# zengjianping/openpose

Hardware: AMD Instinct MI355X
Metric: frames/sec whole-node, BODY_25 -1x368 @1280x720, 1/2/4/8 GPU + CPU ref (higher is better)
Workload: dtype fp16

## Files before the change

openpose_amd/csrc/host/context.h:

```cpp
#pragma once
#include <hip/hip_runtime.h>

#include <map>
#include <memory>
#include <tuple>
#include <vector>

#include "../common.h"
#include "../kernels/kernels.h"
#include "pose_model.h"

struct opk_render_layer;
struct opk_render_heat;

namespace opk {

void cubic_tables(int s, int d, int* ofs, float* coef);

struct Context {
    int device = 0;
    hipStream_t stream = nullptr;
    bool owns_stream = false;

    struct Tables { DevBuf buf; const int* yofs; const float* ycoef; const int* xofs; const float* xcoef; };
    std::map<std::tuple<int, int, int, int>, std::unique_ptr<Tables>> resize_tables;
    const Tables& tables(int sh, int sw, int dh, int dw);

    struct PoseDev { DevBuf buf; PafPairTable t; };
    std::map<int, std::unique_ptr<PoseDev>> pose_dev;
    const PafPairTable& pose_table(int model);

    DevBuf warp_weights[2];
    const short* warp_weight_table(bool cubic);
    struct WarpAxes { DevBuf buf; const int* x; const int* y; };
    std::map<std::tuple<uint64_t, int, int>, std::unique_ptr<WarpAxes>> warp_axes;
    const WarpAxes& warp_axis_tables(double scale, int dw, int dh);

    struct RenderDev { DevBuf buf; const unsigned* pairs; const float* scales; const float* colors;
                       int npairs, nscales, ncolors; };
    std::map<int, std::unique_ptr<RenderDev>> render_dev;
    const RenderDev& render_table(int which);
    DevBuf render_geom;
    DevBuf frames_offsets, frames_keypoints;
    std::vector<int> frames_offsets_host;

    DevBuf scratch_scores;
    DevBuf nms_scratch;
    int* nms_candidates(int frames, int parts);
    HostBuf host_peaks, host_scores;

    std::vector<hipStream_t> side_streams;
    void add_side_stream(hipStream_t s) { side_streams.push_back(s); }
    void remove_side_stream(hipStream_t s)
    {
        for (size_t i = 0; i < side_streams.size(); ++i)
            if (side_streams[i] == s) {
                side_streams.erase(side_streams.begin() + (long)i);
// ... 32 lines not shown
```

openpose_amd/csrc/host/input.cpp:

```cpp
#include "input.h"

#include <cmath>
#include <cstring>
#include <vector>

#include "../common.h"
#include "../kernels/kernels.h"
#include "context.h"

namespace opk {

namespace {
constexpr int kInterBits = 5, kInterTab = 1 << kInterBits;
constexpr int kAbBits = 10, kAbScale = 1 << kAbBits;
constexpr int kCoefScale = 1 << 15;

int round_half_even(double v) { return (int)std::lrint(v); }
int round_half_even(float v) { return (int)std::lrintf(v); }

int positive_round(float v) { return (int)(v + 0.5f); }
int positive_round(double v) { return (int)(v + 0.5f); }
}

void scale_and_size(int in_w, int in_h, int net_w, int net_h, float dyn, int scale_number,
                    double scale_gap, double* scales, int* sizes)
{
    OPK_CHECK_ARG(in_w > 0 && in_h > 0, "Wrong input element (empty cvInputData).");
    OPK_CHECK_ARG(scale_number >= 1, "scale_number must be >= 1");
    if (net_w <= 0 || net_h <= 0) {
// ... 96 lines not shown
        OPK_HIP(hipStreamSynchronize(stream));
    }
    return static_cast<const short*>(b.ptr);
}

const Context::WarpAxes& Context::warp_axis_tables(double scale, int dw, int dh)
{
    uint64_t bits;
    std::memcpy(&bits, &scale, sizeof bits);
    const auto key = std::make_tuple(bits, dw, dh);
    auto it = warp_axes.find(key);
    if (it != warp_axes.end()) return *it->second;
    const bool cubic = scale > 1.;
    std::vector<int> host(2 * (size_t)(dw + dh));
    warp_axis_table(scale, dw, cubic, host.data());
    warp_axis_table(scale, dh, cubic, host.data() + 2 * dw);
    auto t = std::make_unique<WarpAxes>();
    int* dev = static_cast<int*>(t->buf.get(host.size() * sizeof(int)));
    OPK_HIP(hipMemcpyAsync(dev, host.data(), host.size() * sizeof(int), hipMemcpyHostToDevice,
                           stream));
    OPK_HIP(hipStreamSynchronize(stream));
    t->x = dev;
    t->y = dev + 2 * dw;
    auto& ref = *t;
    warp_axes.emplace(key, std::move(t));
    return ref;
}

void cvmat_to_input(Context* ctx, float* dst, const uint8_t* src, int n, int sw, int sh,
                    size_t step, double scale, int dw, int dh, int normalize, hipStream_t stream)
{
    OPK_CHECK_ARG(dst && src, "NULL buffer");
    OPK_CHECK_ARG(n > 0 && sw > 0 && sh > 0 && dw > 0 && dh > 0, "empty frame or net input");
    OPK_CHECK_ARG(scale > 0 && std::isfinite(scale), "scale must be positive");
    ctx->bind();
    const bool cubic = scale > 1.;
    const short* w = ctx->warp_weight_table(cubic);
    const auto& ax = ctx->warp_axis_tables(scale, dw, dh);
    launch_cvmat_to_input(dst, src, n, sh, sw, step ? step : (size_t)sw * 3, dh, dw, ax.x, ax.y, w,
                          cubic ? 4 : 2, normalize, stream ? stream : ctx->stream);
}

}
```

openpose_amd/csrc/host/net.cpp:

```cpp
#include "net.h"

#include "caffemodel.h"

#include <algorithm>
#include <cmath>
#include <cstdlib>
#include <set>

namespace opk {

namespace {
int round_up(int v, int m) { return (v + m - 1) / m * m; }
int pick_bn(int cout)
{
    if (cout <= 32) return 32;
    if (cout <= 64) return 64;
    if (cout <= 96) return 96;
    return 128;
}
}

NetHip::NetHip(Context* ctx, std::vector<LayerDesc> layers, const std::string& output_blob)
    : ctx_(ctx), output_blob_(output_blob)
{
// ... 678 lines not shown
        }
        a.split = S.csplit[ci] ? 1 : 0;
        a.wscale = S.csplit[ci] ? c.wscale : 1.f;
        a.in_lo = S.csplit[ci] && use3 && !S.query[ci].xhi ? S.base_lo[c.in.buf] : nullptr;
        for (size_t q = 0; q < pools_.size(); ++q)
            if (S.poolfused[q] && pool_conv_[q] == (int)ci) {
                a.pool = 1;
                a.ndst = 1;
                a.dst[0] = ptr[pools_[q].out_buf];
                a.dst_lo[0] = S.csplit[ci] ? S.base_lo[pools_[q].out_buf] : nullptr;
                a.dst_cs[0] = bufs_[pools_[q].out_buf].cs;
                a.dst_coff[0] = 0;
            }
        if (c.out32_coff >= 0) {
            OPK_CHECK_ARG(c.level == out_level_, c.info.name + ": output at another resolution");
            a.out32 = S.out32;
            a.out32_c = out_c_;
            a.out32_coff = c.out32_coff;
        }
    }
    return &S;
}

void NetHip::forward(const float* input, int n, int h, int w)
{
    forward_on(input, n, h, w, ctx_->stream, true);
}

float* NetHip::select_output(int n, int h, int w, bool alternate)
{
    OPK_CHECK_ARG(n > 0 && h > 0 && w > 0, "empty input");
    ctx_->bind();
    ShapePlan& S = *shape_plan(n, h, w, ctx_->stream);
    if (alternate) {
        if (!S.out32_alt) {
            const size_t bytes = (size_t)n * out_c_ * S.lh[out_level_] * S.lw[out_level_] * 4;
            S.out32_alt = static_cast<float*>(S.out_mem_alt.get(bytes));
        }
        S.alt = !S.alt;
    }
    return S.out();
}

void NetHip::note_reader(const float* out, hipEvent_t ev)
{
    for (auto& r : readers_)
        if (r.first == out) {
            r.second = ev;
            return;
        }
    readers_.emplace_back(out, ev);
}

void NetHip::forget_reader_events(const hipEvent_t* evs, int n)
{
    for (size_t i = readers_.size(); i-- > 0;)
        for (int k = 0; k < n; ++k)
            if (readers_[i].second == evs[k]) {
                readers_.erase(readers_.begin() + (long)i);
                break;
            }
}

void NetHip::prepare(int n, int h, int w)
{
    OPK_CHECK_ARG(n > 0 && h > 0 && w > 0, "empty input");
    ctx_->bind();
    (void)shape_plan(n, h, w, ctx_->stream);
}

void NetHip::forward_on(const float* input, int n, int h, int w, hipStream_t st, bool timed)
{
    OPK_CHECK_ARG(input && n > 0 && h > 0 && w > 0, "empty input");
    OPK_CHECK_ARG(ready(), "weights not loaded for every convolution");
    ctx_->bind();
    ShapePlan& S = *shape_plan(n, h, w, st);
    cur_ = &S;
    for (const auto& r : readers_)
        if (r.first == S.out()) OPK_HIP(hipStreamWaitEvent(st, r.second, 0));
    if (timed) timer_.begin(st);
    forward_launches(S, input, n, h, w, st);
    if (timed) timer_.end(st);
}

void NetHip::blob(const std::string& name, int f0, int nf, float* host, int shape[4]) const
{
    read_planes(name, f0, nf, nullptr, nullptr, host, shape, nullptr);
}

void NetHip::blob_planes(const std::string& name, int f0, int nf, float* hi, float* lo, int shape[4],
                         int* has_lo) const
{
    read_planes(name, f0, nf, hi, lo, nullptr, shape, has_lo);
}

void NetHip::read_planes(const std::string& name, int f0, int nf, float* hi, float* lo, float* sum,
                         int shape[4], int* has_lo) const
{
    OPK_CHECK_ARG(cur_ != nullptr, "no forward yet");
    const auto it = blob_loc_.find(name);
    OPK_CHECK_ARG(it != blob_loc_.end(), "no blob named " + name);
    const BlobLoc& L = it->second;
    const ShapePlan& S = *cur_;
    OPK_CHECK_ARG(f0 >= 0 && nf > 0 && f0 + nf <= S.n, "frames out of range");
// ... 23 lines not shown
    const size_t frame_elems = (size_t)Hp * Wp * cs;
    std::vector<uint16_t> raw(frame_elems * nf), rlo(twin ? frame_elems * nf : 0);
    OPK_HIP(hipMemcpy(raw.data(), S.base[L.buf] + (size_t)f0 * frame_elems, raw.size() * 2,
                      hipMemcpyDeviceToHost));
    if (twin)
        OPK_HIP(hipMemcpy(rlo.data(), S.base_lo[L.buf] + (size_t)f0 * frame_elems, rlo.size() * 2,
                          hipMemcpyDeviceToHost));
    for (int f = 0; f < nf; ++f)
        for (int y = 0; y < H; ++y)
            for (int x = 0; x < W; ++x) {
                const size_t at = f * frame_elems + ((size_t)(y + B) * Wp + x + B) * cs + L.coff;
                const uint16_t* src = raw.data() + at;
                for (int c = 0; c < L.ch; ++c) {
                    const size_t o = ((size_t)f * L.ch + c) * hw + (size_t)y * W + x;
                    const float vh = (float)__builtin_bit_cast(_Float16, src[c]);
                    const float vl = twin ? (float)__builtin_bit_cast(_Float16, rlo[at + c]) : 0.f;
                    if (hi) hi[o] = vh;
                    if (lo) lo[o] = vl;
                    if (sum) sum[o] = vh + vl;
                }
            }
}

void NetHip::forward_launches(ShapePlan& S, const float* input, int n, int h, int w, hipStream_t st)
{
    const bool logging = dev_switch("LAUNCH_LOG", 0) != 0;
    if (logging) {
        log_.lines.clear();
        attach_launch_log(&log_);
    }
    struct Detach {
        bool on;
        ~Detach() { if (on) attach_launch_log(nullptr); }
    } detach{logging};
    forward_steps(S, input, n, h, w, st);
}

static void launch_conv3_frames(const ConvArgs& a, hipStream_t st)
{
    const int B = a.border > 0 ? a.border : 1;
    Conv3Query q = conv3_query(a);
    const int run = conv3_run_frames(q);
    if (run == a.frames) {
        launch_conv3(a, st);
        return;
    }
    const size_t frame_pos = (size_t)(a.H + 2 * B) * (a.W + 2 * B);
    const size_t dst_pos = a.pool ? (size_t)(a.H / 2 + 2 * B) * (a.W / 2 + 2 * B) : frame_pos;
    for (int f0 = 0; f0 < a.frames; f0 += run) {
        ConvArgs b = a;
        b.frames = std::min(run, a.frames - f0);
        q.frames = b.frames;
        const Conv3Plan pb = conv3_plan(q);
        b.sw = pb.sw;
        b.nstrips = pb.nstrips;
        b.M = b.frames * a.H * (a.W + 2 * B);
        b.in = a.in + f0 * frame_pos * a.in_cs;
        if (a.in_lo) b.in_lo = a.in_lo + f0 * frame_pos * a.in_cs;
        for (int d = 0; d < a.ndst; ++d) {
            b.dst[d] = a.dst[d] + f0 * dst_pos * a.dst_cs[d];
            if (a.dst_lo[d]) b.dst_lo[d] = a.dst_lo[d] + f0 * dst_pos * a.dst_cs[d];
        }
        if (a.out32) b.out32 = a.out32 + (size_t)f0 * a.out32_c * a.H * a.W;
        launch_conv3(b, st);
    }
}

void NetHip::forward_steps(ShapePlan& S, const float* input, int n, int h, int w, hipStream_t st)
{
    LaunchLog* log = launch_log();
    float* const out32 = S.out();
    const std::vector<uint16_t*>& ptr = S.base;
    const std::vector<int>& lh_ = S.lh;
    const std::vector<int>& lw_ = S.lw;
    size_t first = 0;
    if (S.fused1) {
        const ConvPlan& a = convs_[fuse1_.a];
        const ConvPlan& b = convs_[fuse1_.b];
        const PoolPlan& p = pools_[fuse1_.p];
        Conv1FusedArgs fa{};
        fa.img = input;
        fa.frames = n;
        fa.H = h;
        fa.W = w;
        fa.w1 = static_cast<const uint16_t*>(a.w.ptr);
        fa.b1 = static_cast<const float*>(a.bias.ptr);
        fa.s1 = static_cast<const float*>(a.slope.ptr);
        fa.act1 = a.info.act;
        fa.w2 = static_cast<const uint16_t*>(b.w3.ptr);
        fa.b2 = static_cast<const float*>(b.bias.ptr);
        fa.s2 = static_cast<const float*>(b.slope.ptr);
        fa.act2 = b.info.act;
        fa.out = ptr[p.out_buf];
        fa.out_cs = bufs_[p.out_buf].cs;
        fa.out_coff = 0;
        fa.OH = lh_[1];
        fa.OW = lw_[1];
        fa.actmax = a.slope01 && b.slope01 && dev_switch("EPI_MAX", 1) != 0;
        if (log) log->layer = a.info.name + "+" + b.info.name + "+pool";
        launch_conv1_fused(fa, std::min(cus_, std::max(1, dev_switch("GRID_CUS", cus_))), st);
        first = 3;
    }
    for (size_t si = first; si < steps_.size(); ++si) {
        const Step& s = steps_[si];
// ... 118 lines not shown
```

openpose_amd/csrc/host/net.h:

```cpp
#pragma once
#include <map>
#include <memory>
#include <string>
#include <vector>

#include "../kernels/conv.h"
#include "context.h"
#include "graph.h"

namespace opk {

class NetHip {
public:
    NetHip(Context* ctx, std::vector<LayerDesc> layers, const std::string& output_blob = "net_output");

    struct ConvInfo {
        std::string name;
        int cin, cout, k, act;
        std::string act_layer;
    };
    const std::vector<ConvInfo>& convs() const { return info_; }
    void set_conv(const std::string& name, const float* w, const float* b, const float* slope);
    static constexpr int kPrecisionFp16 = 0, kPrecisionSplit = 1;
    void set_precision(int precision);
    void set_precision_schedule(const int* precisions, int count);
    int conv_precision(int index) const;
    void set_small_batch(bool on);
    bool small_batch() const { return small_batch_; }
    void conv_plan(int index, int n, int h, int w, int cus, int* bm, int* bn, int* workgroups,
                   int* small) const;
    std::vector<std::string> conv_kernels(int index, int n, int h, int w, int cus) const;
    bool ready() const;
    int load_caffemodel(const std::string& path);

    void forward(const float* input, int n, int h, int w);
    void forward_on(const float* input, int n, int h, int w, hipStream_t stream, bool timed);
    void prepare(int n, int h, int w);
    void time_begin(hipStream_t s) { timer_.begin(s); }
    void time_end(hipStream_t s) { timer_.end(s); }
    float* output() const { return cur_ ? cur_->out() : nullptr; }
    float* select_output(int n, int h, int w, bool alternate);
    std::weak_ptr<void> liveness() const { return alive_; }
    void note_reader(const float* out, hipEvent_t ev);
    void forget_reader_events(const hipEvent_t* evs, int n);
    int out_channels() const { return out_c_; }
    int out_h() const { return cur_ ? cur_->lh[out_level_] : 0; }
    int out_w() const { return cur_ ? cur_->lw[out_level_] : 0; }
    int frames() const { return cur_ ? cur_->n : 0; }
    static constexpr int kMaxShapes = 8;
    double flops_per_frame(int h, int w) const;
    int border() const { return border_; }
    ~NetHip();

    void set_timing(bool on);
    void read_timing(int* count, double* total_ms);

    void blob(const std::string& name, int f0, int nf, float* host, int shape[4]) const;
    void blob_planes(const std::string& name, int f0, int nf, float* hi, float* lo, int shape[4],
                     int* has_lo) const;
// ... 36 lines not shown
        std::vector<char> headfused;
        std::vector<char> poolfused;
        std::vector<Conv3Query> query;
        std::vector<Conv3Plan> conv;
    };
    Dispatch dispatch(int n, int h, int w, int cus) const;

    struct ShapePlan : Dispatch {
        int n = 0, h = 0, w = 0;
        std::vector<std::unique_ptr<DevBuf>> mem;
        std::vector<uint16_t*> base;
        std::vector<std::unique_ptr<DevBuf>> mem_lo;
        std::vector<uint16_t*> base_lo;
        DevBuf out_mem, out_mem_alt;
        float* out32 = nullptr;
        float* out32_alt = nullptr;
        bool alt = false;
        float* out() const { return alt ? out32_alt : out32; }
        std::vector<ConvArgs> args;
        std::vector<char> use3;
    };

    void plan(const std::vector<LayerDesc>& layers);
    void forward_launches(ShapePlan& S, const float* input, int n, int h, int w, hipStream_t st);
    void forward_steps(ShapePlan& S, const float* input, int n, int h, int w, hipStream_t st);
    ShapePlan* shape_plan(int n, int h, int w, hipStream_t zero_stream = nullptr);

    Context* ctx_;
    std::string output_blob_;
    std::vector<ConvInfo> info_;
    std::vector<ConvPlan> convs_;
    std::map<std::string, int> conv_by_name_;
    std::vector<PoolPlan> pools_;
    std::vector<Step> steps_;
    std::vector<BufSpec> bufs_;
    int out_level_ = 0, out_c_ = 0, nlevels_ = 1;
    int image_buf_ = -1;
    struct Fuse1 { int a = -1, b = -1, p = -1, abuf = -1, bbuf = -1; };
    Fuse1 fuse1_;
    struct FuseHead { int a = -1, b = -1, step = -1, buf = -1; };
    std::vector<FuseHead> heads_;
    std::vector<int> pool_conv_;
    int cus_ = 256;
    bool small_batch_ = false;
    int border_ = 1;

    struct BlobLoc { int buf = -1, coff = 0, ch = 0, level = 0; bool out32 = false; };
    std::map<std::string, BlobLoc> blob_loc_;
// ... 12 lines not shown
```

openpose_amd/csrc/host/pose.cpp:

```cpp
#include "pose.h"

#include <sched.h>

#include <algorithm>
#include <chrono>
#include <cmath>
#include <cstring>
#include <exception>
#include <string>
#include <thread>

#include "../../../include/opk.h"
#include "input.h"
#include "maps.h"

namespace opk {

double resize_scale_factor(int iw, int ih, int tw, int th)
{
    const double rw = (tw - 1) / (double)(iw - 1);
    const double rh = (th - 1) / (double)(ih - 1);
    return rw < rh ? rw : rh;
}

// ... 311 lines not shown
            if (kind == KeypointExtractor::kFace) detect_faces(model_, kp_[f].data(), people_[f], parts, r);
            else detect_hands(model_, kp_[f].data(), people_[f], parts, r);
        }
        p.kp.assign((size_t)per * total * p.ex->parts() * 3, 0.f);
        const double rect_ms =
            std::chrono::duration<double, std::milli>(std::chrono::steady_clock::now() - t0).count();
        p.ex->extract(sl.raw.ptr, sl.raw.n, sl.raw.w, sl.raw.h, sl.raw.step, p.rects.data(),
                      frame_of.data(), total, p.kp.data(), true);
        ++p.batches;
        p.crops += p.ex->crops();
        p.host_ms += rect_ms + p.ex->last_host_ms();
        p.wait_ms += p.ex->last_wait_ms();
    }
    parts_valid_ = true;
}

void PoseHip::submit(const float* frames, int n, int net_h, int net_w, int prod_w, int prod_h)
{
    need_frames();
    OPK_CHECK_ARG(net_ != nullptr, "no network: use forward_net_output (poseNetOutput path)");
    OPK_CHECK_ARG(count_ < 2, "two batches already in flight: collect first");
    ctx_->bind();
    next_output(n, net_h, net_w, true);
    live_net()->forward(frames, n, net_h, net_w);
    const NetOutput o{live_net()->output(), live_net()->out_h(), live_net()->out_w()};
    submit_outputs(&o, 1, n, net_h, net_w, prod_w, prod_h, true);
}

hipStream_t PoseHip::post_stream(bool own_net)
{
    if (!own_net || ctx_->device < 0 || dev_switch("POST_STREAM", 1) == 0) {
        wait_post(ctx_->stream);
        return ctx_->stream;
    }
    if (!post_) {
        OPK_HIP(hipStreamCreateWithFlags(&post_, hipStreamNonBlocking));
        OPK_HIP(hipEventCreateWithFlags(&nets_done_, hipEventDisableTiming));
        for (auto& e : post_done_) OPK_HIP(hipEventCreateWithFlags(&e, hipEventDisableTiming));
        ctx_->add_side_stream(post_);
    }
    OPK_HIP(hipEventRecord(nets_done_, ctx_->stream));
    OPK_HIP(hipStreamWaitEvent(post_, nets_done_, 0));
    return post_;
}

void PoseHip::wait_post(hipStream_t s)
{
// ... 14 lines not shown
    OPK_CHECK_ARG(1. - (scale_number - 1) * scale_gap >= 0. && scale_gap >= 0.,
                  "All scales must be in the range [0, 1], i.e., 0 <= 1-scale_number*scale_gap <= 1");
    in_net_w_ = net_w;
    in_net_h_ = net_h;
    dyn_ = dyn;
    scale_number_ = scale_number;
    scale_gap_ = scale_gap;
}

void PoseHip::submit_frames(const uint8_t* frames, int n, int w, int h, size_t step)
{
    OPK_CHECK_ARG(net_ != nullptr, "no network: raw frames need the net");
    OPK_CHECK_ARG(frames != nullptr && n > 0 && w > 0 && h > 0, "empty frames");
    OPK_CHECK_ARG(count_ < 2, "two batches already in flight: collect first");
    OPK_CHECK_ARG(model_ != 6, "BODY_19N (DenseNet normalisation) is not supported");
    double scales[kMaxResizeSources];
    scale_and_size(w, h, in_net_w_, in_net_h_, dyn_, scale_number_, scale_gap_, scales, input_hw_);
    const float* ptrs[kMaxResizeSources];
    int hw[2 * kMaxResizeSources];
    ctx_->bind();
    for (int i = 0; i < scale_number_; ++i) {
        const int nw = input_hw_[2 * i], nh = input_hw_[2 * i + 1];
        float* x = static_cast<float*>(inputs_[i].get((size_t)n * 3 * nh * nw * sizeof(float)));
        cvmat_to_input(ctx_, x, frames, n, w, h, step, scales[i], nw, nh, 1, ctx_->stream);
        ptrs[i] = x;
        hw[2 * i] = nh;
        hw[2 * i + 1] = nw;
    }
    inputs_n_ = n;
    for (int i = 0; i < scale_number_; ++i) map_ratios_[i] = (float)scales[i];
    have_ratios_ = true;
    cur_raw_ = RawFrames{frames, n, w, h, step};
    try {
        if (scale_number_ == 1)
            submit(ptrs[0], n, hw[0], hw[1], w, h);
        else
            submit_multi(ptrs, hw, scale_number_, n, w, h);
    } catch (...) {
        have_ratios_ = false;
        cur_raw_ = RawFrames{};
        throw;
    }
    have_ratios_ = false;
    cur_raw_ = RawFrames{};
}

void PoseHip::forward_frames(const uint8_t* frames, int n, int w, int h, size_t step)
{
    OPK_CHECK_ARG(count_ == 0, "batches in flight: collect them first");
    submit_frames(frames, n, w, h, step);
    collect();
}

const float* PoseHip::net_input(int i, int* w, int* h) const
{
    OPK_CHECK_ARG(i >= 0 && i < scale_number_ && inputs_n_ > 0, "no such scale");
    if (w) *w = input_hw_[2 * i];
    if (h) *h = input_hw_[2 * i + 1];
    return static_cast<const float*>(inputs_[i].ptr);
}

void PoseHip::submit_multi(const float* const* frames, const int* net_hw, int nscales, int n,
                           int prod_w, int prod_h)
{
    need_frames();
    OPK_CHECK_ARG(net_ != nullptr, "no network: multi-scale needs the net");
    OPK_CHECK_ARG(frames && net_hw && nscales >= 1 && nscales <= kMaxResizeSources,
                  "1..8 scales");
    OPK_CHECK_ARG(count_ < 2, "two batches already in flight: collect first");
    std::vector<NetOutput> outs(nscales);
    for (int i = 0; i < nscales; ++i) OPK_CHECK_ARG(frames[i] != nullptr, "NULL scale input");
    ctx_->bind();
    bool distinct = dev_switch("MULTISCALE_STREAMS", 1) != 0;
    for (int i = 0; i < nscales && distinct; ++i)
        for (int j = 0; j < i; ++j)
            distinct = distinct && !(net_hw[2 * i] == net_hw[2 * j] && net_hw[2 * i + 1] == net_hw[2 * j + 1]);
    for (int i = 0; i < nscales; ++i) next_output(n, net_hw[2 * i], net_hw[2 * i + 1], nscales == 1 || distinct);
    if (nscales == 1 || !distinct) {
        for (int i = 0; i < nscales; ++i) {
            live_net()->forward(frames[i], n, net_hw[2 * i], net_hw[2 * i + 1]);
            outs[i] = NetOutput{live_net()->output(), live_net()->out_h(), live_net()->out_w()};
        }
    } else {
        if (!fork_) {
            OPK_HIP(hipEventCreateWithFlags(&fork_, hipEventDisableTiming));
            for (int i = 0; i < kMaxResizeSources - 1; ++i) {
                OPK_HIP(hipStreamCreateWithFlags(&scale_streams_[i], hipStreamNonBlocking));
                OPK_HIP(hipEventCreateWithFlags(&join_[i], hipEventDisableTiming));
            }
        }
        for (int i = 0; i < nscales; ++i) live_net()->prepare(n, net_hw[2 * i], net_hw[2 * i + 1]);
        hipStream_t s = ctx_->stream;
        live_net()->time_begin(s);
        OPK_HIP(hipEventRecord(fork_, s));
        live_net()->forward_on(frames[0], n, net_hw[0], net_hw[1], s, false);
        outs[0] = NetOutput{live_net()->output(), live_net()->out_h(), live_net()->out_w()};
        for (int i = 1; i < nscales; ++i) {
            OPK_HIP(hipStreamWaitEvent(scale_streams_[i - 1], fork_, 0));
            live_net()->forward_on(frames[i], n, net_hw[2 * i], net_hw[2 * i + 1], scale_streams_[i - 1],
                             false);
            outs[i] = NetOutput{live_net()->output(), live_net()->out_h(), live_net()->out_w()};
            OPK_HIP(hipEventRecord(join_[i - 1], scale_streams_[i - 1]));
        }
        for (int i = 1; i < nscales; ++i) OPK_HIP(hipStreamWaitEvent(s, join_[i - 1], 0));
        live_net()->time_end(s);
    }
    submit_outputs(outs.data(), nscales, n, net_hw[0], net_hw[1], prod_w, prod_h, true);
}

void PoseHip::submit_net_output(const float* net_out, int n, int oh, int ow, int net_h,
                                int net_w, int prod_w, int prod_h)
{
    need_frames();
    const NetOutput o{net_out, oh, ow};
    submit_outputs(&o, 1, n, net_h, net_w, prod_w, prod_h, false);
}

void PoseHip::submit_outputs(const NetOutput* outs, int nscales, int n, int net_h, int net_w,
                             int prod_w, int prod_h, bool own_net)
{
    const PoseModelInfo& m = pose_model(model_);
    const int C = m.heat_channels();
    OPK_CHECK_ARG(n > 0 && nscales >= 1 && nscales <= kMaxResizeSources, "bad batch");
// ... 227 lines not shown
```

openpose_amd/csrc/host/pose.h:

```cpp
#pragma once
#include <memory>
#include <vector>

#include "connector.h"
#include "context.h"
#include "extract.h"
#include "net.h"
#include "pool.h"

namespace opk {

class PoseHip {
public:
    PoseHip(Context* ctx, NetHip* net, bool maximize_positives, int pose_model = 0,
            int semantics = kConnectCpu);
    ~PoseHip();

    void set_property(int prop, double v);
    void set_map_semantics(int maps);
    int map_semantics() const { return maps_; }
    double property(int prop) const { return props_[prop]; }
    void set_overlay(const float* overlay) { overlay_ = overlay; }
    void set_upsampling_ratio(float ratio);
    float upsampling_ratio() const { return upsampling_; }
// ... 57 lines not shown
    struct Slot {
        DevBuf peaks, records;
        HostBuf hpeaks, hrecords;
        hipEvent_t done = nullptr;
        int n = 0, H = 0, W = 0;
        float scale = 1.f;
        HeatMap heat{};
        RawFrames raw{};
    };
    struct Part {
        KeypointExtractor* ex = nullptr;
        std::weak_ptr<void> alive;
        int parts = 0;
        std::vector<Rect> rects;
        std::vector<float> kp;
        int batches = 0, crops = 0;
        double host_ms = 0., wait_ms = 0.;
    };
    Part part_[2];
    DevBuf part_dev_[2];
    std::vector<int> part_first_;
    bool parts_valid_ = false;
    RawFrames cur_raw_{};
    bool any_attached() const { return attached(0) || attached(1); }
    void need_frames() const;
    void run_parts(const Slot& sl);
    struct NetOutput {
        const float* ptr;
        int h, w;
    };
    void submit_outputs(const NetOutput* outs, int nscales, int n, int net_h, int net_w,
                        int prod_w, int prod_h, bool own_net);
    size_t record_floats() const;

    Context* ctx_;
    NetHip* net_;
    std::weak_ptr<void> net_alive_;
    NetHip* live_net() const;
    int in_net_w_ = -1, in_net_h_ = 368, scale_number_ = 1;
    float dyn_ = 1.f;
    double scale_gap_ = 0.25;
    DevBuf inputs_[kMaxResizeSources];
    int input_hw_[2 * kMaxResizeSources] = {};
    int inputs_n_ = 0;
    bool maximize_positives_;
    int model_, semantics_;
// ... 40 lines not shown
```

openpose_amd/csrc/kernels/conv.h:

```cpp
#pragma once
#include <hip/hip_runtime.h>

#include <cstdint>

namespace opk {

constexpr int kConvMaxDst = 6;
constexpr int kConvBK = 64;

struct ConvArgs {
    const uint16_t* in;
    int in_cs, in_coff;
    int cin_pad;
    int ntaps;
    int tapoff[9];
    int ksteps;
    const uint16_t* w;
    const float* bias;
    const float* slope;
    int act;
    int frames, H, W;
    int M;
    int cout;
    int ndst;
// ... 101 lines not shown
    int split;
    const uint16_t* in_lo;
    uint16_t* dst_lo[kConvMaxDst];
    float wscale6, wscale7;
};
bool conv_head_supported(int n1, int n2, int cin_pad);
void conv_head_pack_w7(uint16_t* dst, const uint16_t* w7 , int n1, int n2);
void launch_conv_head(const HeadArgs& a, hipStream_t stream);

void launch_conv_image(const ConvArgs& a, const float* image, hipStream_t stream);

struct Conv1FusedArgs {
    const float* img;
    int frames, H, W;
    const uint16_t* w1;
    const float *b1, *s1;
    int act1;
    const uint16_t* w2;
    const float *b2, *s2;
    int act2;
    uint16_t* out;
    int out_cs, out_coff, OH, OW;
    int actmax;
};
bool conv1_fused_supported(int H, int W, int cout1, int cout2);
void launch_conv1_fused(const Conv1FusedArgs& a, int workgroups, hipStream_t stream);

void launch_maxpool2_split(uint16_t* out, uint16_t* out_lo, const uint16_t* in, const uint16_t* in_lo,
                           int frames, int H, int W, int C, int OH, int OW, hipStream_t stream,
                           int border);
void launch_maxpool2(uint16_t* out, const uint16_t* in, int frames, int H, int W, int C, int OH,
                     int OW, hipStream_t stream, int border = 1);

}
```

openpose_amd/csrc/kernels/conv1_fused.hip:

```cpp
#include "conv.h"

#include <algorithm>

#include "../common.h"
#include "conv3_dev.h"

namespace opk {

namespace {

typedef _Float16 half8_t __attribute__((ext_vector_type(8)));
typedef _Float16 half2_t __attribute__((ext_vector_type(2)));
typedef float float4_t __attribute__((ext_vector_type(4)));
typedef float float2_t __attribute__((ext_vector_type(2)));

#ifndef OPK1_ABLATE
#define OPK1_ABLATE 0
#endif

constexpr int TR = 6, TC = 62, VW = 64;
constexpr int MT = TR * VW;
constexpr int HROWS = (TR + 2) * VW + 8;
constexpr int PR = TR + 4, PCW = TC + 4;
constexpr int PATCH = 3 * PR * PCW;
constexpr int PC = 67, PS = 683, PD = 2072;
static_assert(PC >= PCW && PS >= PR * PC && PC % 32 == 3 && PS % 32 == 11 && PD % 32 == 24, "patch layout");
constexpr int PATCH_LDS = PD + 3 * PS;
constexpr int NT = 512;
constexpr int PPL = (PATCH + NT - 1) / NT;
constexpr int TSTRIDE = 72;
constexpr int W2_PIECES = 18 * 64 * 4;
constexpr int HALO_PIECES = 2 * HROWS * 4;
constexpr int LDS_BYTES = (W2_PIECES + HALO_PIECES) * 16 + (PATCH_LDS * 4 + 15) / 16 * 16;
static_assert(MT * TSTRIDE * 2 <= HALO_PIECES * 16, "epilogue tile fits in the halo");
static_assert(LDS_BYTES <= 160 * 1024, "LDS budget");

__device__ __forceinline__ int swz64(int row, int piece) { return row * 4 + (piece ^ (((row >> 2) & 1) << 1)); }
__device__ __forceinline__ int swzh(int row, int piece) { return row * 4 + (piece ^ ((row >> 1) & 3)); }

__device__ __forceinline__ uint32_t hmax4(uint32_t a, uint32_t b, uint32_t c, uint32_t d)
{
    const half2_t m = __builtin_elementwise_max(
        __builtin_elementwise_max(__builtin_bit_cast(half2_t, a), __builtin_bit_cast(half2_t, b)),
        __builtin_elementwise_max(__builtin_bit_cast(half2_t, c), __builtin_bit_cast(half2_t, d)));
    return __builtin_bit_cast(uint32_t, m);
}

template <bool MX>
__global__ __launch_bounds__(NT, 1) void conv1_fused_kernel(const Conv1FusedArgs a)
{
    __shared__ uint4 lds[LDS_BYTES / 16];
    uint4* W2 = lds;
    uint4* HALO = lds + W2_PIECES;
    float* patch = reinterpret_cast<float*>(lds + W2_PIECES + HALO_PIECES);
    uint16_t* T = reinterpret_cast<uint16_t*>(HALO);

    const int tid = threadIdx.x, lane = tid & 63;
    const int wave = __builtin_amdgcn_readfirstlane(tid >> 6);
    const int r16 = lane & 15, q = lane >> 4;
    const int H = a.H, W = a.W;
    const int tiles_x = (W + TC - 1) / TC, tiles_y = (H + TR - 1) / TR;
    const int ntiles = a.frames * tiles_x * tiles_y;

    {
        const int lrow = lane >> 2, phys = lane & 3;
#pragma unroll
        for (int k = 0; k < W2_PIECES / NT; ++k) {
            const int inst = k * 8 + wave;
            const int row = inst * 16 + lrow;
            const int lp = phys ^ (((row >> 2) & 1) << 1);
            __builtin_amdgcn_global_load_lds((const void*)(a.w2 + (size_t)row * 32 + lp * 8),
                                             (__attribute__((address_space(3))) void*)(&W2[inst * 64]),
                                             16, 0, 0);
        }
    }
    half8_t w1f[4];
    float4_t b1[4], m1[4], b2[4], m2[4];
    const float neg1 = a.act1 == 1 ? 0.f : 1.f, neg2 = a.act2 == 1 ? 0.f : 1.f;
// ... 30 lines not shown
        x0_ = tx_ * TC;                                                                       \
    } while (0)
    float pre[PPL];
#define OPK1_LOAD_PATCH(tile_)                                                                \
    do {                                                                                      \
        int f_, y0_, x0_;                                                                     \
        OPK1_ORIGIN(tile_, f_, y0_, x0_);                                                     \
        const float* src_ = a.img + (size_t)f_ * 3 * H * W;                                   \
        _Pragma("unroll") for (int k_ = 0; k_ < PPL; ++k_) {                                  \
            const int i_ = tid + k_ * NT;                                                     \
            float v_ = 0.f;                                                                   \
            if (i_ < PATCH && (tile_) < ntiles) {                                             \
                const int ci_ = i_ / (PR * PCW);                                              \
                const int rem_ = i_ - ci_ * (PR * PCW);                                       \
                const int r_ = rem_ / PCW, c_ = rem_ - (rem_ / PCW) * PCW;                    \
                const int y_ = y0_ - 2 + r_, x_ = x0_ - 2 + c_;                               \
                if (y_ >= 0 && y_ < H && x_ >= 0 && x_ < W)                                   \
                    v_ = src_[((size_t)ci_ * H + y_) * W + x_];                               \
            }                                                                                 \
            pre[k_] = v_;                                                                     \
        }                                                                                     \
    } while (0)

    int pool_dp, pool_cg;
    {
        const unsigned g1m = 0xF00F0FF0u;
        const int lo = lane & 31;
        const bool g1 = (g1m >> lo) & 1u;
        const unsigned same = g1 ? g1m : ~g1m;
        const int k = __popc(same & ((1u << lo) - 1u));
        pool_dp = (g1 ? 1 : 0) + 2 * (lane >> 5) + 4 * (k >> 3);
        pool_cg = k & 7;
    }

    int pli[PPL];
#pragma unroll
    for (int k = 0; k < PPL; ++k) {
        const int i = tid + k * NT;
        const int ci = i / (PR * PCW), rem = i - ci * (PR * PCW);
        const int r = rem / PCW, cc = rem - r * PCW;
        pli[k] = i < PATCH ? ci * PS + r * PC + cc : -1;
    }

    int tile = blockIdx.x;
    OPK1_LOAD_PATCH(tile);
    for (; tile < ntiles; tile += gridDim.x) {
        int f, y0, x0;
        OPK1_ORIGIN(tile, f, y0, x0);
        __syncthreads();
#pragma unroll
        for (int k = 0; k < PPL; ++k)
            if (pli[k] >= 0) {
                patch[pli[k]] = pre[k];
                patch[PD + pli[k]] = pre[k];
            }
        asm volatile("s_waitcnt vmcnt(0)" ::: "memory");
        __syncthreads();

        float xv[4][8];
#pragma unroll
        for (int gi = 0; gi < 4; ++gi) {
            const int mh = (wave * 4 + gi) * 16 + r16;
            const int base = (mh >> 6) * PC + (mh & 63);
#pragma unroll
            for (int e = 0; e < 8; ++e) xv[gi][e] = patch[off[e] + base];
        }
        float4_t c1[4][4];
#pragma unroll
        for (int gi = 0; gi < 4; ++gi) {
            half8_t xf;
#pragma unroll
            for (int e = 0; e < 8; ++e)
                xf[e] = OPK1_ABLATE == 1 ? (_Float16)0.f
                        : ((kvalid >> e) & 1u) ? (_Float16)xv[gi][e] : (_Float16)0.f;
#pragma unroll
            for (int g = 0; g < 4; ++g)
                c1[gi][g] = OPK1_ABLATE == 1 ? float4_t{(float)xf[0], 0.f, 0.f, 0.f}
                    : __builtin_amdgcn_mfma_f32_16x16x32_f16(w1f[g], xf, float4_t{0.f, 0.f, 0.f, 0.f},
                                                             0, 0, 0);
// ... 2 lines not shown
        for (int gi = 0; gi < 4; ++gi) {
            const int mh = (wave * 4 + gi) * 16 + r16;
            const int hr = mh >> 6, hc = mh & 63;
            const int y = y0 - 1 + hr, x = x0 - 1 + hc;
            const bool in = y >= 0 && y < H && x >= 0 && x < W;
            uint32_t pk[4][2];
#pragma unroll
            for (int g = 0; g < 4; ++g) {
                const float4_t t = c1[gi][g] + b1[g];
                const float4_t a_ = conv3dev::act_pick4<MX>(t, t * m1[g]);
                const float4_t v = in ? a_ : float4_t{0.f, 0.f, 0.f, 0.f};
                pk[g][0] = __builtin_bit_cast(uint32_t, __builtin_convertvector(v.xy, half2_t));
                pk[g][1] = __builtin_bit_cast(uint32_t, __builtin_convertvector(v.zw, half2_t));
            }
#pragma unroll
            for (int c = 0; c < 2; ++c) {
                const auto sl = __builtin_amdgcn_permlane16_swap(pk[2 * c][0], pk[2 * c + 1][0], false, false);
                const auto sh = __builtin_amdgcn_permlane16_swap(pk[2 * c][1], pk[2 * c + 1][1], false, false);
                HALO[c * HROWS * 4 + swzh(mh, 2 * (q & 1) + (q >> 1))] = make_uint4(sl[0], sh[0], sl[1], sh[1]);
            }
        }
        __syncthreads();

        OPK1_LOAD_PATCH(tile + gridDim.x);
        float4_t acc[3][4];
#pragma unroll
        for (int i = 0; i < 3; ++i)
#pragma unroll
            for (int j = 0; j < 4; ++j) acc[i][j] = float4_t{0.f, 0.f, 0.f, 0.f};
        half8_t fa[2][3], fb[2][4];
#define OPK1_READ(buf_, st_)                                                                  \
    do {                                                                                      \
        const int c_ = (st_) / 9, tap_ = (st_) - 9 * ((st_) / 9);                             \
        const int ky_ = tap_ / 3, kx_ = tap_ - 3 * (tap_ / 3);                                \
        const uint4* As_ = HALO + c_ * HROWS * 4;                                             \
        const uint4* Bs_ = W2 + (c_ * 9 + tap_) * 256;                                        \
        _Pragma("unroll") for (int i_ = 0; i_ < 3; ++i_)                                      \
            fa[buf_][i_] = __builtin_bit_cast(                                                \
                half8_t, As_[swzh(wave * 48 + i_ * 16 + r16 + ky_ * VW + kx_, q)]);             \
        _Pragma("unroll") for (int j_ = 0; j_ < 4; ++j_)                                      \
            fb[buf_][j_] = __builtin_bit_cast(half8_t, Bs_[swz64(j_ * 16 + r16, q)]);           \
    } while (0)
        OPK1_READ(0, 0);
#pragma unroll
        for (int st = 0; st < 18; ++st) {
            const int cur = st & 1;
            if (st + 1 < 18) OPK1_READ(cur ^ 1, st + 1);
// ... 42 lines not shown

        for (int it = wave; it < (TR / 2) * 4; it += NT / 64) {
            const int slot = it * 8 + pool_dp;
            const int cg = pool_cg;
            const int pr = slot >> 5, pc = slot & 31;
            const int oy = y0 / 2 + pr, ox = x0 / 2 + pc;
            if (pc >= TC / 2 || 2 * oy + 1 >= H || 2 * ox + 1 >= W) continue;
            const int m0 = (2 * pr) * VW + 2 * pc;
            const uint16_t* s0 = T + m0 * TSTRIDE + cg * 8;
            uint4 v0 = *reinterpret_cast<const uint4*>(s0);
            const uint4 v1 = *reinterpret_cast<const uint4*>(s0 + TSTRIDE);
            const uint4 v2 = *reinterpret_cast<const uint4*>(s0 + VW * TSTRIDE);
            const uint4 v3 = *reinterpret_cast<const uint4*>(s0 + (VW + 1) * TSTRIDE);
            v0.x = hmax4(v0.x, v1.x, v2.x, v3.x);
            v0.y = hmax4(v0.y, v1.y, v2.y, v3.y);
            v0.z = hmax4(v0.z, v1.z, v2.z, v3.z);
            v0.w = hmax4(v0.w, v1.w, v2.w, v3.w);
            uint16_t* dst = a.out + (((size_t)f * (a.OH + 2) + oy + 1) * (a.OW + 2) + ox + 1) * a.out_cs +
                            a.out_coff + cg * 8;
            *reinterpret_cast<uint4*>(dst) = v0;
        }
    }
#undef OPK1_LOAD_PATCH
#undef OPK1_ORIGIN
}

}

bool conv1_fused_supported(int H, int W, int cout1, int cout2)
{
    return cout1 == 64 && cout2 == 64 && H % 2 == 0 && W % 2 == 0 && H >= 2 && W >= 2;
}

void launch_conv1_fused(const Conv1FusedArgs& a, int workgroups, hipStream_t stream)
{
    OPK_CHECK_ARG(a.img && a.w1 && a.w2 && a.out && a.b1 && a.b2 && a.s1 && a.s2, "NULL argument");
    OPK_CHECK_ARG(a.frames > 0 && conv1_fused_supported(a.H, a.W, 64, 64), "conv1 fusion: sizes");
    OPK_CHECK_ARG(a.OH == a.H / 2 && a.OW == a.W / 2, "conv1 fusion: pooled size");
    OPK_CHECK_ARG(a.out_cs % 8 == 0 && a.out_coff % 8 == 0 && a.out_coff + 64 <= a.out_cs,
                  "conv1 fusion: 16-byte aligned output slice");
    const long tiles = (long)a.frames * ((a.W + TC - 1) / TC) * ((a.H + TR - 1) / TR);
    OPK_CHECK_ARG(tiles < (1L << 31), "conv1 fusion: too many tiles");
    const int grid = (int)std::min<long>(tiles, workgroups > 0 ? workgroups : 256);
    note_launch("%s<%d>", kConv1FusedKernel, a.actmax ? 1 : 0);
    if (a.actmax) hipLaunchKernelGGL(conv1_fused_kernel<true>, dim3(grid), dim3(NT), 0, stream, a);
    else hipLaunchKernelGGL(conv1_fused_kernel<false>, dim3(grid), dim3(NT), 0, stream, a);
    OPK_LAUNCH_CHECK();
}

}
```

Measured before the change: 3793.

## Fuse bilinear frame warp into the fused conv1 kernel input loads

The fused conv1 kernel can now read raw uint8 BGR frames and do the bilinear warp itself, using packed 16-bit axis tables held in LDS. This replaces the separate cvmat_to_input resize kernel and its float input round trip through memory. The warped input is still written to img_out for the tiles' interior pixels so later consumers keep working. The cost is more LDS, extra per-pixel gather and interpolation work inside the conv kernel, and a new path limited to linear warps whose tables fit in 16 bits.

Measured after the change: 3821 (median of 6 runs). About the same (+0.8%).

```diff
diff --git a/openpose_amd/csrc/host/context.h b/openpose_amd/csrc/host/context.h
--- a/openpose_amd/csrc/host/context.h
+++ b/openpose_amd/csrc/host/context.h
@@ -32,7 +32,7 @@
 
     DevBuf warp_weights[2];
     const short* warp_weight_table(bool cubic);
-    struct WarpAxes { DevBuf buf; const int* x; const int* y; };
+    struct WarpAxes { DevBuf buf; const int* x; const int* y; bool pack16; };
     std::map<std::tuple<uint64_t, int, int>, std::unique_ptr<WarpAxes>> warp_axes;
     const WarpAxes& warp_axis_tables(double scale, int dw, int dh);
 
diff --git a/openpose_amd/csrc/host/input.cpp b/openpose_amd/csrc/host/input.cpp
--- a/openpose_amd/csrc/host/input.cpp
+++ b/openpose_amd/csrc/host/input.cpp
@@ -5,6 +5,7 @@
 #include <vector>
 
 #include "../common.h"
+#include "../kernels/conv.h"
 #include "../kernels/kernels.h"
 #include "context.h"
 
@@ -147,6 +148,7 @@
     OPK_HIP(hipStreamSynchronize(stream));
     t->x = dev;
     t->y = dev + 2 * dw;
+    t->pack16 = !cubic && conv1_fused_warp_tables_fit(host.data(), dw, host.data() + 2 * dw, dh);
     auto& ref = *t;
     warp_axes.emplace(key, std::move(t));
     return ref;
diff --git a/openpose_amd/csrc/host/net.cpp b/openpose_amd/csrc/host/net.cpp
--- a/openpose_amd/csrc/host/net.cpp
+++ b/openpose_amd/csrc/host/net.cpp
@@ -724,9 +724,19 @@
     return &S;
 }
 
-void NetHip::forward(const float* input, int n, int h, int w)
-{
-    forward_on(input, n, h, w, ctx_->stream, true);
+void NetHip::forward(const float* input, int n, int h, int w, const FrameSource* frames)
+{
+    forward_on(input, n, h, w, ctx_->stream, true, frames);
+}
+
+bool NetHip::takes_frames(const FrameSource& fs, int n, int h, int w)
+{
+    OPK_CHECK_ARG(n > 0 && h > 0 && w > 0, "empty input");
+    if (dev_switch("CONV1_WARP", 1) == 0 || !fs.frames || !(fs.scale > 0.) || fs.scale > 1.) return false;
+    if (!conv1_fused_warp_supported(h, w, fs.h, fs.w)) return false;
+    ctx_->bind();
+    if (!shape_plan(n, h, w, ctx_->stream)->fused1) return false;
+    return ctx_->warp_axis_tables(fs.scale, w, h).pack16;
 }
 
 float* NetHip::select_output(int n, int h, int w, bool alternate)
@@ -771,7 +781,8 @@
     (void)shape_plan(n, h, w, ctx_->stream);
 }
 
-void NetHip::forward_on(const float* input, int n, int h, int w, hipStream_t st, bool timed)
+void NetHip::forward_on(const float* input, int n, int h, int w, hipStream_t st, bool timed,
+                        const FrameSource* frames)
 {
     OPK_CHECK_ARG(input && n > 0 && h > 0 && w > 0, "empty input");
     OPK_CHECK_ARG(ready(), "weights not loaded for every convolution");
@@ -781,7 +792,7 @@
     for (const auto& r : readers_)
         if (r.first == S.out()) OPK_HIP(hipStreamWaitEvent(st, r.second, 0));
     if (timed) timer_.begin(st);
-    forward_launches(S, input, n, h, w, st);
+    forward_launches(S, input, n, h, w, st, frames);
     if (timed) timer_.end(st);
 }
 
@@ -851,7 +862,8 @@
             }
 }
 
-void NetHip::forward_launches(ShapePlan& S, const float* input, int n, int h, int w, hipStream_t st)
+void NetHip::forward_launches(ShapePlan& S, const float* input, int n, int h, int w, hipStream_t st,
+                              const FrameSource* frames)
 {
     const bool logging = dev_switch("LAUNCH_LOG", 0) != 0;
     if (logging) {
@@ -862,7 +874,7 @@
         bool on;
         ~Detach() { if (on) attach_launch_log(nullptr); }
     } detach{logging};
-    forward_steps(S, input, n, h, w, st);
+    forward_steps(S, input, n, h, w, st, frames);
 }
 
 static void launch_conv3_frames(const ConvArgs& a, hipStream_t st)
@@ -895,8 +907,10 @@
     }
 }
 
-void NetHip::forward_steps(ShapePlan& S, const float* input, int n, int h, int w, hipStream_t st)
-{
+void NetHip::forward_steps(ShapePlan& S, const float* input, int n, int h, int w, hipStream_t st,
+                           const FrameSource* frames)
+{
+    OPK_CHECK_ARG(!frames || S.fused1, "a frame source needs the fused conv1 unit (takes_frames)");
     LaunchLog* log = launch_log();
     float* const out32 = S.out();
     const std::vector<uint16_t*>& ptr = S.base;
@@ -909,6 +923,20 @@
         const PoolPlan& p = pools_[fuse1_.p];
         Conv1FusedArgs fa{};
         fa.img = input;
+        if (frames) {
+            const auto& ax = ctx_->warp_axis_tables(frames->scale, w, h);
+            OPK_CHECK_ARG(frames->scale <= 1. && ax.pack16, "frame source: not a linear warp that fits");
+            fa.img = nullptr;
+            fa.img_out = const_cast<float*>(input);
+            fa.src = frames->frames;
+            fa.sh = frames->h;
+            fa.sw = frames->w;
+            fa.src_step = frames->step ? frames->step : (size_t)frames->w * 3;
+            fa.src_frame = fa.src_step * frames->h;
+            fa.xtab = ax.x;
+            fa.ytab = ax.y;
+            fa.wtab = ctx_->warp_weight_table(false);
+        }
         fa.frames = n;
         fa.H = h;
         fa.W = w;
diff --git a/openpose_amd/csrc/host/net.h b/openpose_amd/csrc/host/net.h
--- a/openpose_amd/csrc/host/net.h
+++ b/openpose_amd/csrc/host/net.h
@@ -9,6 +9,13 @@
 #include "graph.h"
 
 namespace opk {
+
+struct FrameSource {
+    const uint8_t* frames;
+    int w, h;
+    size_t step;
+    double scale;
+};
 
 class NetHip {
 public:
@@ -33,8 +40,10 @@
     bool ready() const;
     int load_caffemodel(const std::string& path);
 
-    void forward(const float* input, int n, int h, int w);
-    void forward_on(const float* input, int n, int h, int w, hipStream_t stream, bool timed);
+    void forward(const float* input, int n, int h, int w, const FrameSource* frames = nullptr);
+    void forward_on(const float* input, int n, int h, int w, hipStream_t stream, bool timed,
+                    const FrameSource* frames = nullptr);
+    bool takes_frames(const FrameSource& frames, int n, int h, int w);
     void prepare(int n, int h, int w);
     void time_begin(hipStream_t s) { timer_.begin(s); }
     void time_end(hipStream_t s) { timer_.end(s); }
@@ -117,8 +126,10 @@
     };
 
     void plan(const std::vector<LayerDesc>& layers);
-    void forward_launches(ShapePlan& S, const float* input, int n, int h, int w, hipStream_t st);
-    void forward_steps(ShapePlan& S, const float* input, int n, int h, int w, hipStream_t st);
+    void forward_launches(ShapePlan& S, const float* input, int n, int h, int w, hipStream_t st,
+                          const FrameSource* frames);
+    void forward_steps(ShapePlan& S, const float* input, int n, int h, int w, hipStream_t st,
+                       const FrameSource* frames);
     ShapePlan* shape_plan(int n, int h, int w, hipStream_t zero_stream = nullptr);
 
     Context* ctx_;
diff --git a/openpose_amd/csrc/host/pose.cpp b/openpose_amd/csrc/host/pose.cpp
--- a/openpose_amd/csrc/host/pose.cpp
+++ b/openpose_amd/csrc/host/pose.cpp
@@ -357,7 +357,7 @@
     OPK_CHECK_ARG(count_ < 2, "two batches already in flight: collect first");
     ctx_->bind();
     next_output(n, net_h, net_w, true);
-    live_net()->forward(frames, n, net_h, net_w);
+    live_net()->forward(frames, n, net_h, net_w, scale_source(0));
     const NetOutput o{live_net()->output(), live_net()->out_h(), live_net()->out_w()};
     submit_outputs(&o, 1, n, net_h, net_w, prod_w, prod_h, true);
 }
@@ -418,7 +418,10 @@
     for (int i = 0; i < scale_number_; ++i) {
         const int nw = input_hw_[2 * i], nh = input_hw_[2 * i + 1];
         float* x = static_cast<float*>(inputs_[i].get((size_t)n * 3 * nh * nw * sizeof(float)));
-        cvmat_to_input(ctx_, x, frames, n, w, h, step, scales[i], nw, nh, 1, ctx_->stream);
+        cur_src_[i] = FrameSource{frames, w, h, step, scales[i]};
+        cur_fused_[i] = live_net()->takes_frames(cur_src_[i], n, nh, nw);
+        if (!cur_fused_[i])
+            cvmat_to_input(ctx_, x, frames, n, w, h, step, scales[i], nw, nh, 1, ctx_->stream);
         ptrs[i] = x;
         hw[2 * i] = nh;
         hw[2 * i + 1] = nw;
@@ -435,10 +438,12 @@
     } catch (...) {
         have_ratios_ = false;
         cur_raw_ = RawFrames{};
+        std::fill(cur_fused_, cur_fused_ + kMaxResizeSources, false);
         throw;
     }
     have_ratios_ = false;
     cur_raw_ = RawFrames{};
+    std::fill(cur_fused_, cur_fused_ + kMaxResizeSources, false);
 }
 
 void PoseHip::forward_frames(const uint8_t* frames, int n, int w, int h, size_t step)
@@ -474,7 +479,7 @@
     for (int i = 0; i < nscales; ++i) next_output(n, net_hw[2 * i], net_hw[2 * i + 1], nscales == 1 || distinct);
     if (nscales == 1 || !distinct) {
         for (int i = 0; i < nscales; ++i) {
-            live_net()->forward(frames[i], n, net_hw[2 * i], net_hw[2 * i + 1]);
+            live_net()->forward(frames[i], n, net_hw[2 * i], net_hw[2 * i + 1], scale_source(i));
             outs[i] = NetOutput{live_net()->output(), live_net()->out_h(), live_net()->out_w()};
         }
     } else {
@@ -489,12 +494,12 @@
         hipStream_t s = ctx_->stream;
         live_net()->time_begin(s);
         OPK_HIP(hipEventRecord(fork_, s));
-        live_net()->forward_on(frames[0], n, net_hw[0], net_hw[1], s, false);
+        live_net()->forward_on(frames[0], n, net_hw[0], net_hw[1], s, false, scale_source(0));
         outs[0] = NetOutput{live_net()->output(), live_net()->out_h(), live_net()->out_w()};
         for (int i = 1; i < nscales; ++i) {
             OPK_HIP(hipStreamWaitEvent(scale_streams_[i - 1], fork_, 0));
             live_net()->forward_on(frames[i], n, net_hw[2 * i], net_hw[2 * i + 1], scale_streams_[i - 1],
-                             false);
+                             false, scale_source(i));
             outs[i] = NetOutput{live_net()->output(), live_net()->out_h(), live_net()->out_w()};
             OPK_HIP(hipEventRecord(join_[i - 1], scale_streams_[i - 1]));
         }
diff --git a/openpose_amd/csrc/host/pose.h b/openpose_amd/csrc/host/pose.h
--- a/openpose_amd/csrc/host/pose.h
+++ b/openpose_amd/csrc/host/pose.h
@@ -103,6 +103,9 @@
     std::vector<int> part_first_;
     bool parts_valid_ = false;
     RawFrames cur_raw_{};
+    FrameSource cur_src_[kMaxResizeSources] = {};
+    bool cur_fused_[kMaxResizeSources] = {};
+    const FrameSource* scale_source(int i) const { return cur_fused_[i] ? &cur_src_[i] : nullptr; }
     bool any_attached() const { return attached(0) || attached(1); }
     void need_frames() const;
     void run_parts(const Slot& sl);
diff --git a/openpose_amd/csrc/kernels/conv.h b/openpose_amd/csrc/kernels/conv.h
--- a/openpose_amd/csrc/kernels/conv.h
+++ b/openpose_amd/csrc/kernels/conv.h
@@ -147,8 +147,16 @@
     uint16_t* out;
     int out_cs, out_coff, OH, OW;
     int actmax;
+    const uint8_t* src;
+    int sh, sw;
+    size_t src_step, src_frame;
+    const int *xtab, *ytab;
+    const short* wtab;
+    float* img_out;
 };
 bool conv1_fused_supported(int H, int W, int cout1, int cout2);
+bool conv1_fused_warp_supported(int H, int W, int sh, int sw);
+bool conv1_fused_warp_tables_fit(const int* xtab, int W, const int* ytab, int H);
 void launch_conv1_fused(const Conv1FusedArgs& a, int workgroups, hipStream_t stream);
 
 void launch_maxpool2_split(uint16_t* out, uint16_t* out_lo, const uint16_t* in, const uint16_t* in_lo,
diff --git a/openpose_amd/csrc/kernels/conv1_fused.hip b/openpose_amd/csrc/kernels/conv1_fused.hip
--- a/openpose_amd/csrc/kernels/conv1_fused.hip
+++ b/openpose_amd/csrc/kernels/conv1_fused.hip
@@ -4,6 +4,7 @@
 
 #include "../common.h"
 #include "conv3_dev.h"
+#include "warp_dev.h"
 
 namespace opk {
 
@@ -34,6 +35,10 @@
 constexpr int LDS_BYTES = (W2_PIECES + HALO_PIECES) * 16 + (PATCH_LDS * 4 + 15) / 16 * 16;
 static_assert(MT * TSTRIDE * 2 <= HALO_PIECES * 16, "epilogue tile fits in the halo");
 static_assert(LDS_BYTES <= 160 * 1024, "LDS budget");
+constexpr int TAB_MAX = 3520;
+static_assert(LDS_BYTES + TAB_MAX * 2 <= 160 * 1024 && TAB_MAX % 8 == 0, "LDS budget with the tables");
+constexpr int TAP_MAX = (1 << 11) - 1;
+constexpr int PPX = (PR * PCW + NT - 1) / NT;
 
 __device__ __forceinline__ int swz64(int row, int piece) { return row * 4 + (piece ^ (((row >> 2) & 1) << 1)); }
 __device__ __forceinline__ int swzh(int row, int piece) { return row * 4 + (piece ^ ((row >> 1) & 3)); }
@@ -46,14 +51,15 @@
     return __builtin_bit_cast(uint32_t, m);
 }
 
-template <bool MX>
+template <bool MX, bool WARP>
 __global__ __launch_bounds__(NT, 1) void conv1_fused_kernel(const Conv1FusedArgs a)
 {
-    __shared__ uint4 lds[LDS_BYTES / 16];
+    __shared__ uint4 lds[(LDS_BYTES + (WARP ? TAB_MAX * 2 : 0)) / 16];
     uint4* W2 = lds;
     uint4* HALO = lds + W2_PIECES;
     float* patch = reinterpret_cast<float*>(lds + W2_PIECES + HALO_PIECES);
     uint16_t* T = reinterpret_cast<uint16_t*>(HALO);
+    uint16_t* tab16 = reinterpret_cast<uint16_t*>(lds + LDS_BYTES / 16);
 
     const int tid = threadIdx.x, lane = tid & 63;
     const int wave = __builtin_amdgcn_readfirstlane(tid >> 6);
@@ -130,6 +136,38 @@
         }                                                                                     \
     } while (0)
 
+    uint32_t went[PPX] = {}, wlo[PPX][2] = {}, whi[PPX][2] = {};
+    uint2 wwt[PPX] = {};
+#define OPK1_LOAD_TAPS(tile_)                                                                 \
+    do {                                                                                      \
+        if ((tile_) < ntiles) {                                                               \
+            int f_, y0_, x0_;                                                                 \
+            OPK1_ORIGIN(tile_, f_, y0_, x0_);                                                 \
+            const uint8_t* fsrc_ = a.src + (size_t)f_ * a.src_frame;                          \
+            _Pragma("unroll") for (int k_ = 0; k_ < PPX; ++k_) {                              \
+                const int i_ = tid + k_ * NT;                                                 \
+                if (i_ < PR * PCW) {                                                          \
+                    const int r_ = i_ / PCW, c_ = i_ - (i_ / PCW) * PCW;                      \
+                    const int y_ = min(max(y0_ - 2 + r_, 0), H - 1);                          \
+                    const int x_ = min(max(x0_ - 2 + c_, 0), W - 1);                          \
+                    const uint32_t xe_ = tab16[x_], ye_ = tab16[W + y_];                      \
+                    went[k_] = ye_ << 16 | xe_;                                               \
+                    wwt[k_] = *reinterpret_cast<const uint2*>(                                \
+                        a.wtab + ((ye_ & 31) * 32 + (xe_ & 31)) * 4);                         \
+                    const int xs_ = min((int)(xe_ >> 5), a.sw - 2);                           \
+                    _Pragma("unroll") for (int ky_ = 0; ky_ < 2; ++ky_) {                     \
+                        const int yy_ = min((int)(ye_ >> 5) + ky_, a.sh - 1);                 \
+                        const uint8_t* p_ = fsrc_ + (size_t)yy_ * a.src_step + xs_ * 3;       \
+                        uint16_t h_;                                                          \
+                        __builtin_memcpy(&wlo[k_][ky_], p_, 4);                               \
+                        __builtin_memcpy(&h_, p_ + 4, 2);                                     \
+                        whi[k_][ky_] = h_;                                                    \
+                    }                                                                         \
+                }                                                                             \
+            }                                                                                 \
+        }                                                                                     \
+    } while (0)
+
     int pool_dp, pool_cg;
     {
         const unsigned g1m = 0xF00F0FF0u;
@@ -151,18 +189,69 @@
     }
 
     int tile = blockIdx.x;
-    OPK1_LOAD_PATCH(tile);
+    if constexpr (WARP) {
+        const int2* xt = reinterpret_cast<const int2*>(a.xtab);
+        const int2* yt = reinterpret_cast<const int2*>(a.ytab);
+        for (int i = tid; i < W + H; i += NT) {
+            const int2 e = i < W ? xt[i] : yt[i - W];
+            tab16[i] = (uint16_t)(e.x << 5 | e.y);
+        }
+        __syncthreads();
+        OPK1_LOAD_TAPS(tile);
+    } else {
+        OPK1_LOAD_PATCH(tile);
+    }
     for (; tile < ntiles; tile += gridDim.x) {
         int f, y0, x0;
         OPK1_ORIGIN(tile, f, y0, x0);
         __syncthreads();
-#pragma unroll
-        for (int k = 0; k < PPL; ++k)
-            if (pli[k] >= 0) {
-                patch[pli[k]] = pre[k];
-                patch[PD + pli[k]] = pre[k];
+        if constexpr (WARP) {
+#pragma unroll
+            for (int k = 0; k < PPX; ++k) {
+                const int i = tid + k * NT;
+                if (i >= PR * PCW) continue;
+                const int r = i / PCW, c = i - r * PCW;
+                const int y = y0 - 2 + r, x = x0 - 2 + c;
+                float v[3] = {0.f, 0.f, 0.f};
+                if (y >= 0 && y < H && x >= 0 && x < W) {
+                    const int xtap = (went[k] & 0xffffu) >> 5, ytap = went[k] >> 21;
+                    uint8_t raw[2][6];
+#pragma unroll
+                    for (int ky = 0; ky < 2; ++ky) {
+                        uint64_t b = (uint64_t)whi[k][ky] << 32 | wlo[k][ky];
+                        if (xtap > a.sw - 2) b >>= 24;
+#pragma unroll
+                        for (int j = 0; j < 6; ++j) raw[ky][j] = (uint8_t)(b >> (8 * j));
+                    }
+                    const short wk[4] = {(short)(wwt[k].x & 0xffffu), (short)(wwt[k].x >> 16),
+                                         (short)(wwt[k].y & 0xffffu), (short)(wwt[k].y >> 16)};
+                    int u[3];
+                    warp_pixel<2>(u, int2{0, (int)(went[k] >> 16 & 31u)}, int2{0, (int)(went[k] & 31u)},
+                                  wk, a.sh - ytap, a.sw - xtap, [&](int ky, int) { return raw[ky]; });
+#pragma unroll
+                    for (int ci = 0; ci < 3; ++ci) v[ci] = (float)u[ci] * (1.f / 256.f) - 0.5f;
+                    if (a.img_out && r >= 2 && r < 2 + TR && c >= 2 && c < 2 + TC) {
+                        float* o = a.img_out + ((size_t)f * 3 * H + y) * W + x;
+#pragma unroll
+                        for (int ci = 0; ci < 3; ++ci) o[(size_t)ci * H * W] = v[ci];
+                    }
+                }
+#pragma unroll
+                for (int ci = 0; ci < 3; ++ci) {
+                    patch[ci * PS + r * PC + c] = v[ci];
+                    patch[PD + ci * PS + r * PC + c] = v[ci];
+                }
             }
-        asm volatile("s_waitcnt vmcnt(0)" ::: "memory");
+            if (tile == (int)blockIdx.x) asm volatile("s_waitcnt vmcnt(0)" ::: "memory");
+        } else {
+#pragma unroll
+            for (int k = 0; k < PPL; ++k)
+                if (pli[k] >= 0) {
+                    patch[pli[k]] = pre[k];
+                    patch[PD + pli[k]] = pre[k];
+                }
+            asm volatile("s_waitcnt vmcnt(0)" ::: "memory");
+        }
         __syncthreads();
 
         float xv[4][8];
@@ -211,7 +300,8 @@
         }
         __syncthreads();
 
-        OPK1_LOAD_PATCH(tile + gridDim.x);
+        if constexpr (WARP) OPK1_LOAD_TAPS(tile + gridDim.x);
+        else OPK1_LOAD_PATCH(tile + gridDim.x);
         float4_t acc[3][4];
 #pragma unroll
         for (int i = 0; i < 3; ++i)
@@ -300,6 +390,7 @@
         }
     }
 #undef OPK1_LOAD_PATCH
+#undef OPK1_LOAD_TAPS
 #undef OPK1_ORIGIN
 }
 
@@ -310,9 +401,30 @@
     return cout1 == 64 && cout2 == 64 && H % 2 == 0 && W % 2 == 0 && H >= 2 && W >= 2;
 }
 
+bool conv1_fused_warp_supported(int H, int W, int sh, int sw)
+{
+    return H + W <= TAB_MAX && sh >= 1 && sw >= 2 && sh <= TAP_MAX && sw <= TAP_MAX;
+}
+
+bool conv1_fused_warp_tables_fit(const int* xtab, int W, const int* ytab, int H)
+{
+    for (int i = 0; i < W + H; ++i) {
+        const int* e = i < W ? xtab + 2 * i : ytab + 2 * (i - W);
+        if (e[0] < 0 || e[0] > TAP_MAX || e[1] < 0 || e[1] > 31) return false;
+    }
+    return true;
+}
+
 void launch_conv1_fused(const Conv1FusedArgs& a, int workgroups, hipStream_t stream)
 {
-    OPK_CHECK_ARG(a.img && a.w1 && a.w2 && a.out && a.b1 && a.b2 && a.s1 && a.s2, "NULL argument");
+    OPK_CHECK_ARG((a.img || a.src) && a.w1 && a.w2 && a.out && a.b1 && a.b2 && a.s1 && a.s2,
+                  "NULL argument");
+    if (a.src) {
+        OPK_CHECK_ARG(a.xtab && a.ytab && a.wtab, "conv1 fusion: NULL warp table");
+        OPK_CHECK_ARG(conv1_fused_warp_supported(a.H, a.W, a.sh, a.sw), "conv1 fusion: warp sizes");
+        OPK_CHECK_ARG(a.src_step >= (size_t)a.sw * 3 && a.src_frame >= a.src_step * (a.sh - 1) + (size_t)a.sw * 3,
+                      "conv1 fusion: row or frame step shorter than the data");
+    }
     OPK_CHECK_ARG(a.frames > 0 && conv1_fused_supported(a.H, a.W, 64, 64), "conv1 fusion: sizes");
     OPK_CHECK_ARG(a.OH == a.H / 2 && a.OW == a.W / 2, "conv1 fusion: pooled size");
     OPK_CHECK_ARG(a.out_cs % 8 == 0 && a.out_coff % 8 == 0 && a.out_coff + 64 <= a.out_cs,
@@ -320,9 +432,16 @@
     const long tiles = (long)a.frames * ((a.W + TC - 1) / TC) * ((a.H + TR - 1) / TR);
     OPK_CHECK_ARG(tiles < (1L << 31), "conv1 fusion: too many tiles");
     const int grid = (int)std::min<long>(tiles, workgroups > 0 ? workgroups : 256);
+    if (a.src) {
+        note_launch("%s<%d,warp>", kConv1FusedKernel, a.actmax ? 1 : 0);
+        if (a.actmax) hipLaunchKernelGGL((conv1_fused_kernel<true, true>), dim3(grid), dim3(NT), 0, stream, a);
+        else hipLaunchKernelGGL((conv1_fused_kernel<false, true>), dim3(grid), dim3(NT), 0, stream, a);
+        OPK_LAUNCH_CHECK();
+        return;
+    }
     note_launch("%s<%d>", kConv1FusedKernel, a.actmax ? 1 : 0);
-    if (a.actmax) hipLaunchKernelGGL(conv1_fused_kernel<true>, dim3(grid), dim3(NT), 0, stream, a);
-    else hipLaunchKernelGGL(conv1_fused_kernel<false>, dim3(grid), dim3(NT), 0, stream, a);
+    if (a.actmax) hipLaunchKernelGGL((conv1_fused_kernel<true, false>), dim3(grid), dim3(NT), 0, stream, a);
+    else hipLaunchKernelGGL((conv1_fused_kernel<false, false>), dim3(grid), dim3(NT), 0, stream, a);
     OPK_LAUNCH_CHECK();
 }
 
```
